# liulisixin/MLI-NeRF

Hardware: AMD Instinct MI355X
Metric: rays/sec + PSNR, syn_hotdog 4096 rays x128 samples, 1/2/4/8 MI355X (higher is better)
Workload: dtype fp16; 1 GPU; syn_hotdog_b stage-b train step; rays_per_gpu=4096, samples_per_ray=128, global_rays=4096, parallelism=dp1, pipeline=geometry prefetch on a side stream, gate heads, 2 batch(es) ahead, output_layer_dw=forward partials (pq), tail=fused, reductions=ordered

## Files before the change

mli_nerf_amd/csrc/params.hip:

```cpp
#include "common.h"

namespace {

__global__ __launch_bounds__(256) void row_scale_kernel(const mli_pack_layer* layers, float* row_scale) {
  const mli_pack_layer& L = layers[blockIdx.y];
  const int row = blockIdx.x * 4 + (threadIdx.x >> 6), lane = threadIdx.x & 63;
  if (row >= L.n_out) return;
  const float* vr = L.v + (size_t)row * L.k_ref;
  float ss = 0.f;
  for (int k = lane; k < L.k_ref; k += 64) ss += vr[k] * vr[k];
#pragma unroll
  for (int o = 32; o > 0; o >>= 1) ss += __shfl_xor(ss, o);
  if (lane == 0) row_scale[blockIdx.y * 256 + row] = L.g[row] / sqrtf(ss);
}

__global__ __launch_bounds__(256) void pack_kernel(const mli_pack_layer* layers, uint8_t* dst,
                                                   const float* row_scale) {
  const mli_pack_layer& L = layers[blockIdx.y];
  const float* rs = row_scale + blockIdx.y * 256;
  const int per_tile = (L.k_steps + 1) * 64;
  const int gid = blockIdx.x * blockDim.x + threadIdx.x;
  if (gid >= L.n_tiles * per_tile) return;
  const int t = gid / per_tile, rem = gid - t * per_tile;
  const int q = rem >> 6, lane = rem & 63;
  uint8_t* chunk = dst + L.dst_offset + (size_t)t * L.chunk_stride;
  const int rows_src = L.n_out, cols_src = L.k_ref;
  if (q == L.k_steps) {
    if (lane >= 32) return;
    const int hh = lane >> 4, i = lane & 15;
    const int n = 32 * t + acc_row(i, hh);
    float b = 0.f;
    if (!L.transpose && L.bias && n < rows_src) b = L.bias[n];
    reinterpret_cast<float*>(chunk + L.k_steps * 1024)[hh * 16 + i] = b;
    return;
  }
  const int rl = lane & 31, hh = lane >> 5;
  const int n = 32 * t + rl;
  half8 out;
  const float sc_row = (!L.transpose && n < rows_src) ? rs[n] : 0.f;
#pragma unroll
  for (int j = 0; j < 8; ++j) {
    const int kk = L.kmode[q] ? k_acc(q, hh, j) : k_nat(q, hh, j);
    const int src = L.kmap[kk];
    float w = 0.f;
    if (src >= 0) {
      if (!L.transpose) {
        if (n < rows_src) w = L.v[(size_t)n * cols_src + src] * sc_row;
      } else {
        const int col = L.nmap ? L.nmap[n] : (n < cols_src ? n : -1);
        if (col >= 0) w = L.v[(size_t)src * cols_src + col] * rs[src];
      }
    }
    out[j] = (f16)w;
  }
  *reinterpret_cast<half8*>(chunk + q * 1024 + lane * 16) = out;
}

__global__ __launch_bounds__(256) void assemble_kernel(const mli_assemble_layer* layers, float inv_scale,
                                                       int zero_dw) {
  const mli_assemble_layer& L = layers[blockIdx.y];
  const int n = blockIdx.x;
  if (n >= L.n_out) return;
  __shared__ float red[2][256];
  const int tid = threadIdx.x;
  float* dwz = const_cast<float*>(L.dw);
  if (L.plain) {
    for (int c = tid; c < L.k_ref; c += 256) {
      const size_t i = (size_t)n * L.k_pack + L.kinv[c];
      L.grad_v[(size_t)n * L.k_ref + c] = L.dw[i] * inv_scale;
      if (zero_dw) dwz[i] = 0.f;
    }
    if (tid == 0) {
      L.grad_b[n] = L.db[n] * inv_scale;
      if (zero_dw) const_cast<float*>(L.db)[n] = 0.f;
    }
    return;
  }
  const float* vr = L.v + (size_t)n * L.k_ref;
  float ss = 0.f, dot = 0.f;
  for (int c = tid; c < L.k_ref; c += 256) {
    const float d = L.dw[(size_t)n * L.k_pack + L.kinv[c]] * inv_scale;
    ss += vr[c] * vr[c];
    dot += d * vr[c];
  }
  red[0][tid] = ss;
  red[1][tid] = dot;
  __syncthreads();
  for (int s = 128; s > 0; s >>= 1) {
    if (tid < s) {
      red[0][tid] += red[0][tid + s];
      red[1][tid] += red[1][tid + s];
    }
    __syncthreads();
  }
  const float nrm = sqrtf(red[0][0]);
  const float dg = red[1][0] / nrm;
  const float gs = L.g[n] / nrm;
  for (int c = tid; c < L.k_ref; c += 256) {
    const size_t i = (size_t)n * L.k_pack + L.kinv[c];
    const float d = L.dw[i] * inv_scale;
    L.grad_v[(size_t)n * L.k_ref + c] = gs * (d - dg * vr[c] / nrm);
    if (zero_dw) dwz[i] = 0.f;
  }
  if (tid == 0) {
    L.grad_g[n] = dg;
    L.grad_b[n] = L.db[n] * inv_scale;
    if (zero_dw) const_cast<float*>(L.db)[n] = 0.f;
  }
}

struct AdamwCoef {
  float decay, omb1, beta2, omb2, step_size, bc2_sqrt, eps;
};

__device__ __forceinline__ void adamw_one(const AdamwCoef& c, float& p, float g, float& m, float& v) {
  p = p * c.decay;
  m = m + (g - m) * c.omb1;
  v = v * c.beta2 + (g * g) * c.omb2;
  const float denom = sqrtf(v) / c.bc2_sqrt + c.eps;
  p = p - c.step_size * (m / denom);
}

__global__ __launch_bounds__(256) void adamw_kernel(mli_adamw_args a, AdamwCoef c) {
  const int64_t i = (int64_t)blockIdx.x * blockDim.x + threadIdx.x;
  if (i >= a.n) return;
  float p = a.p[i], m = a.m[i], v = a.v[i];
  const float g = a.g[i];
  adamw_one(c, p, g, m, v);
  a.p[i] = p;
  a.m[i] = m;
  a.v[i] = v;
  if (a.p16) a.p16[i] = __builtin_bit_cast(uint16_t, (f16)p);
  if (a.zero_grad && g != 0.0f) a.g[i] = 0.0f;
}

__global__ __launch_bounds__(256) void cast_kernel(mli_cast_args a) {
  const int64_t i = (int64_t)blockIdx.x * blockDim.x + threadIdx.x;
  if (i >= a.n) return;
  a.dst[i] = __builtin_bit_cast(uint16_t, (f16)a.src[i]);
}

}

extern "C" int mli_pack(const mli_pack_args* a, mli_stream_t s) {
  const int max_threads = 8 * (19 + 1) * 64;
  if (a->n_layers <= 0) return 0;
  if (a->row_scale == nullptr) return (int)hipErrorInvalidValue;
  hipLaunchKernelGGL(row_scale_kernel, dim3(64, a->n_layers), dim3(256), 0, (hipStream_t)s, a->layers,
                     a->row_scale);
  hipLaunchKernelGGL(pack_kernel, dim3((max_threads + 255) / 256, a->n_layers), dim3(256), 0,
                     (hipStream_t)s, a->layers, a->dst, (const float*)a->row_scale);
  MLI_LAUNCH_CHECK();
}

extern "C" int mli_pack_workspace(const mli_pack_args* a, int64_t* bytes) {
  bytes[0] = (int64_t)(a->n_layers > 0 ? a->n_layers : 0) * 256 * 4;
  return 0;
}

extern "C" int mli_grad_assemble(const mli_assemble_args* a, mli_stream_t s) {
  hipLaunchKernelGGL(assemble_kernel, dim3(256, a->n_layers), dim3(256), 0, (hipStream_t)s,
                     a->layers, a->inv_scale, a->zero_dw);
  MLI_LAUNCH_CHECK();
}

extern "C" int mli_adamw(const mli_adamw_args* a, mli_stream_t s) {
  if (a->n <= 0) return 0;
  const double bc1 = 1.0 - pow(a->beta1, (double)a->step);
  const double bc2 = 1.0 - pow(a->beta2, (double)a->step);
  const AdamwCoef c = {(float)(1.0 - a->lr * a->weight_decay), (float)(1.0 - a->beta1), (float)a->beta2,
                       (float)(1.0 - a->beta2), (float)(a->lr / bc1), (float)sqrt(bc2), (float)a->eps};
  hipLaunchKernelGGL(adamw_kernel, dim3((unsigned)((a->n + 255) / 256)), dim3(256), 0, (hipStream_t)s, *a, c);
  MLI_LAUNCH_CHECK();
}

extern "C" int mli_cast_f16(const mli_cast_args* a, mli_stream_t s) {
  if (a->n <= 0) return 0;
  hipLaunchKernelGGL(cast_kernel, dim3((unsigned)((a->n + 255) / 256)), dim3(256), 0, (hipStream_t)s, *a);
  MLI_LAUNCH_CHECK();
}

extern "C" int mli_abi_version(void) { return MLI_ABI_VERSION; }

#ifndef MLI_SOURCE_HASH
#define MLI_SOURCE_HASH "unknown"
#endif
static const char mli_source_hash_tag[] __attribute__((used)) = "MLI_SOURCE_HASH=" MLI_SOURCE_HASH;
extern "C" const char* mli_source_hash(void) { return mli_source_hash_tag + 16; }

extern "C" const char* mli_error_string(int code) { return hipGetErrorString((hipError_t)code); }
```

mli_nerf_amd/csrc/rays.hip:

```cpp
#include "common.h"
#include "loss.h"
#include "mli_relight.h"

namespace {

MLI_FI float light_pos(const float* Q, int i) {
  return -((Q[4 * 0 + i] * Q[3] + Q[4 * 1 + i] * Q[7]) + Q[4 * 2 + i] * Q[11]);
}

__global__ __launch_bounds__(256) void rays_kernel(mli_rays_args a) {
  const int r = blockIdx.x * blockDim.x + threadIdx.x;
  if (r >= a.R) return;
  const int64_t pix = a.ray_idx ? a.ray_idx[r] : a.first_pixel + r;
  const float py = (float)(pix / a.W) + 0.5f;
  const float px = (float)(pix % a.W) + 0.5f;
  float K[9], T[12], TL[3];
  {
    const float* M = a.intr;
    const float c00 = M[4] * M[8] - M[5] * M[7], c01 = M[5] * M[6] - M[3] * M[8], c02 = M[3] * M[7] - M[4] * M[6];
    const float det = (M[0] * c00 + M[1] * c01) + M[2] * c02;
    const float id = 1.0f / det;
    K[0] = c00 * id; K[1] = (M[2] * M[7] - M[1] * M[8]) * id; K[2] = (M[1] * M[5] - M[2] * M[4]) * id;
    K[3] = c01 * id; K[4] = (M[0] * M[8] - M[2] * M[6]) * id; K[5] = (M[2] * M[3] - M[0] * M[5]) * id;
    K[6] = c02 * id; K[7] = (M[1] * M[6] - M[0] * M[7]) * id; K[8] = (M[0] * M[4] - M[1] * M[3]) * id;
// ... 455 lines not shown
  for (int o = 16; o > 0; o >>= 1) t += __shfl_xor(t, o);
  if (j == 0) fin[i] = t;
  __syncthreads();
  if (threadIdx.x == 0) mli_loss::finalize(L, fin);
}

__global__ __launch_bounds__(256) void composite_bwd_kernel(mli_composite_bwd_args a) {
  const int R = a.R;
  const size_t S = (size_t)R * a.N;
  const size_t s = (size_t)blockIdx.x * 256 + threadIdx.x;
  if (s >= S) return;
  const int r = (int)(s % (size_t)R);
  float dr[3], dor[3], dre[3], orr[3];
  for (int i = 0; i < 3; ++i) {
    dre[i] = a.d_o_re ? a.d_o_re[3 * r + i] : 0.f;
    dr[i] = a.d_rgb ? a.d_rgb[3 * r + i] : 0.f;
    dor[i] = a.d_o_r ? a.d_o_r[3 * r + i] : 0.f;
    orr[i] = a.o_r[3 * r + i];
  }
  const float dos = a.d_o_s ? a.d_o_s[r] : 0.f;
  const f32x4 y0 = *reinterpret_cast<const f32x4*>(a.y + 8 * s);
  const f32x4 y1 = *reinterpret_cast<const f32x4*>(a.y + 8 * s + 4);
  const float y[7] = {y0[0], y0[1], y0[2], y0[3], y1[0], y1[1], y1[2]};
  float D[7];
  ray_dz(dr, dor, dos, dre, orr, a.o_s[r], D);
  if (a.dray && s < (size_t)R) store_dray(a.dray, r, D);
  f32x4 o0, o1;
  composite_bwd_sample(D, a.weights[s] * a.grad_scale, y, o0, o1);
  *reinterpret_cast<f32x4*>(a.dz4 + 8 * s) = o0;
  *reinterpret_cast<f32x4*>(a.dz4 + 8 * s + 4) = o1;
}


__global__ __launch_bounds__(CW * 64) void composite_bwd_geo_kernel(mli_composite_bwd_geo_args a) {
  const int lane = threadIdx.x & 63, w = threadIdx.x >> 6;
  const int R = a.R, N = a.N;
  const int r = blockIdx.x * CW + w;
  if (r >= R) return;
  const float inv_s = expf(a.s_var[0]);
  const float an = a.anneal;
  const float v0 = a.ray_unit[3 * r], v1 = a.ray_unit[3 * r + 1], v2 = a.ray_unit[3 * r + 2];
  const float far = a.far_[r];
  const float dr0 = a.d_rgb[3 * r], dr1 = a.d_rgb[3 * r + 1], dr2 = a.d_rgb[3 * r + 2];
  const float bg = a.white_bg ? (dr0 + dr1) + dr2 : 0.f;
  constexpr int E = 4;
  float al[E], x[E], cp[E], cn[E], ep[E], en[E], st[E], cs[E], dw[E], yv[E][3];
  float lp = 1.f;
#pragma unroll
  for (int e = 0; e < E; ++e) {
    const int k = E * lane + e;
    al[e] = 0.f; x[e] = 0.f; cp[e] = cn[e] = 0.5f; ep[e] = en[e] = 0.f; st[e] = 0.f; cs[e] = 0.f; dw[e] = 0.f;
    yv[e][0] = yv[e][1] = yv[e][2] = 0.f;
    if (k < N) {
      const size_t s = (size_t)k * R + r;
      const float dk = a.dists[s];
      const float dn = (k + 1 < N) ? a.dists[s + R] : far;
      st[e] = dn - dk;
      const float g0 = a.grad[3 * s], g1 = a.grad[3 * s + 1], g2 = a.grad[3 * s + 2];
      cs[e] = (v0 * g0 + v1 * g1) + v2 * g2;
      const float ic = -(fmaxf(-cs[e] * 0.5f + 0.5f, 0.f) * (1.0f - an) + fmaxf(-cs[e], 0.f) * an);
      const float sd = a.sdf[s];
      ep[e] = sd - (ic * st[e]) * 0.5f;
      en[e] = sd + (ic * st[e]) * 0.5f;
      cp[e] = 1.0f / (1.0f + expf(-(ep[e] * inv_s)));
      cn[e] = 1.0f / (1.0f + expf(-(en[e] * inv_s)));
      x[e] = (cp[e] - cn[e]) / (cp[e] + 1e-5f);
      al[e] = fminf(fmaxf(x[e], 0.f), 1.f);
      const f32x4 y0 = *reinterpret_cast<const f32x4*>(a.y + 8 * s);
      yv[e][0] = y0[0]; yv[e][1] = y0[1]; yv[e][2] = y0[2];
      dw[e] = ((dr0 * y0[0] + dr1 * y0[1]) + dr2 * y0[2]) - bg;
    }
    lp *= 1.0f - al[e];
  }
  float T[E];
  T[0] = wave_excl_prod(lp, lane);
#pragma unroll
  for (int e = 1; e < E; ++e) T[e] = T[e - 1] * (1.0f - al[e - 1]);
  float ma = 1.f, mb = 0.f;
#pragma unroll
  for (int e = E - 1; e >= 0; --e) {
    mb = (1.0f - al[e]) * mb + dw[e] * al[e];
    ma = (1.0f - al[e]) * ma;
  }
#pragma unroll
  for (int o = 1; o < 64; o <<= 1) {
    const float na = __shfl_down(ma, o), nb = __shfl_down(mb, o);
    if (lane + o < 64) { mb = ma * nb + mb; ma = ma * na; }
  }
  float B = __shfl_down(mb, 1);
  if (lane == 63) B = 0.f;
  float dinv = 0.f;
#pragma unroll
  for (int e = E - 1; e >= 0; --e) {
    const int k = E * lane + e;
    const float da = T[e] * (dw[e] - B);
    B = (1.0f - al[e]) * B + dw[e] * al[e];
    if (k >= N) continue;
    const size_t s = (size_t)k * R + r;
    const float dx = (x[e] >= 0.f && x[e] <= 1.f) ? da : 0.f;
    const float den_ = cp[e] + 1e-5f;
    const float dcp = dx * (1.0f - x[e]) / den_, dcn = -dx / den_;
    const float dtp = dcp * (cp[e] * (1.0f - cp[e])), dtn = dcn * (cn[e] * (1.0f - cn[e]));
    const float dep = dtp * inv_s, den = dtn * inv_s;
    dinv += dtp * ep[e] + dtn * en[e];
    a.d_sdf[s] = dep + den;
    const float dic = (den - dep) * 0.5f * st[e];
    const float dcos = dic * ((-cs[e] * 0.5f + 0.5f > 0.f ? 0.5f * (1.0f - an) : 0.f) + (-cs[e] > 0.f ? an : 0.f));
    a.d_grad[3 * s] = v0 * dcos;
    a.d_grad[3 * s + 1] = v1 * dcos;
    a.d_grad[3 * s + 2] = v2 * dcos;
    const float wsc = al[e] * T[e] * a.grad_scale;
    f32x4 o0, o1;
    o0[0] = wsc * dr0 * (yv[e][0] * (1.f - yv[e][0]));
    o0[1] = wsc * dr1 * (yv[e][1] * (1.f - yv[e][1]));
    o0[2] = wsc * dr2 * (yv[e][2] * (1.f - yv[e][2]));
    o0[3] = 0.f;
    o1[0] = o1[1] = o1[2] = o1[3] = 0.f;
    *reinterpret_cast<f32x4*>(a.dz4 + 8 * s) = o0;
    *reinterpret_cast<f32x4*>(a.dz4 + 8 * s + 4) = o1;
  }
  dinv = wave_sum(dinv);
  if (lane == 0) a.d_inv_s_part[r] = dinv;
}

__global__ __launch_bounds__(256) void svar_grad_kernel(mli_composite_bwd_geo_args a) {
  __shared__ float red[256];
  float t = 0.f;
  for (int r = threadIdx.x; r < a.R; r += 256) t += a.d_inv_s_part[r];
  red[threadIdx.x] = t;
  __syncthreads();
  for (int o = 128; o > 0; o >>= 1) {
    if ((int)threadIdx.x < o) red[threadIdx.x] += red[threadIdx.x + o];
    __syncthreads();
  }
  if (threadIdx.x == 0) a.d_s_var[0] = expf(a.s_var[0]) * red[0];
}


MLI_FI uint32_t mix32(uint32_t x) {
  x ^= x >> 16; x *= 0x7feb352du; x ^= x >> 15; x *= 0x846ca68bu; x ^= x >> 16;
  return x;
}

MLI_FI uint64_t feistel(uint64_t x, int bits, uint64_t seed) {
  const int lb = bits >> 1, hb = bits - lb;
  const uint64_t lmask = (1ull << lb) - 1ull, hmask = (1ull << hb) - 1ull;
  uint64_t L = x >> lb, Rr = x & lmask;
  for (int k = 0; k < 4; ++k) {
    const uint32_t f = mix32((uint32_t)Rr ^ mix32((uint32_t)(seed >> (8 * k)) + 0x9e3779b9u * (k + 1)) ^
                             (uint32_t)(seed >> 32));
    const uint64_t nL = Rr, nR = (L ^ f) & hmask;
    const uint64_t comb = (nL << hb) | nR;
    L = comb >> lb;
    Rr = comb & lmask;
  }
  return (L << lb) | Rr;
}

__global__ __launch_bounds__(256) void ray_batch_kernel(mli_ray_batch_args a) {
  const int r = blockIdx.x * blockDim.x + threadIdx.x;
  if (r >= a.R) return;
  int bits = 1;
  while ((1ll << bits) < a.n_pixels) ++bits;
  uint64_t x = (uint64_t)r;
  do {
    x = feistel(x, bits, a.seed);
  } while (x >= (uint64_t)a.n_pixels);
  const int64_t p = (int64_t)x, n = a.n_pixels;
  a.ray_idx[r] = p;
  if (a.image)
    for (int c = 0; c < 3; ++c) a.image_sampled[3 * r + c] = a.image[c * n + p];
  if (a.ref)
    for (int c = 0; c < 3; ++c) a.ref_sampled[3 * r + c] = a.ref[c * n + p];
  if (a.sha) a.sha_sampled[r] = a.sha[p];
  if (a.cert) a.cert_sampled[r] = a.cert[p];
}

}

extern "C" int mli_rays(const mli_rays_args* a, mli_stream_t s) {
  if (a->R <= 0) return 0;
  hipLaunchKernelGGL(rays_kernel, dim3((a->R + 255) / 256), dim3(256), 0, (hipStream_t)s, *a);
  MLI_LAUNCH_CHECK();
}

extern "C" int mli_light_points(const mli_light_points_args* a, mli_stream_t s) {
  if (a->L <= 0 || a->R <= 0) return 0;
  if (!a->pose_lights || !a->pts_light) return (int)hipErrorInvalidValue;
  if ((int64_t)a->L * a->R > INT32_MAX) return (int)hipErrorInvalidValue;
  const int64_t n = (int64_t)a->L * a->R * 3;
  hipLaunchKernelGGL(light_points_kernel, dim3((unsigned)((n + 255) / 256)), dim3(256), 0, (hipStream_t)s, *a);
  MLI_LAUNCH_CHECK();
}

extern "C" int mli_sample_coarse(const mli_sample_coarse_args* a, mli_stream_t s) {
  const int n = a->R * a->Nc;
  if (n <= 0) return 0;
  hipLaunchKernelGGL(sample_coarse_kernel, dim3((n + 255) / 256), dim3(256), 0, (hipStream_t)s, *a);
  MLI_LAUNCH_CHECK();
}

extern "C" int mli_sample_fine(const mli_sample_fine_args* a, mli_stream_t s) {
  if (a->R <= 0) return 0;
  if (a->Nf > FBMAX || a->Nb > FBMAX || a->Na < 1 || a->Na + a->Nb > FMAX) return (int)hipErrorInvalidValue;
  if (a->Nf > 0 && a->sdf_out == nullptr) return (int)hipErrorInvalidValue;
  if ((a->inside_list == nullptr) != (a->n_inside == nullptr)) return (int)hipErrorInvalidValue;
  FineArgs fa;
  fa.a = *a;
  for (int j = 0; j < 64; ++j) fa.u[j] = (j < a->Nf && a->u_fine) ? a->u_fine[j] : 2.0f;
  hipLaunchKernelGGL(sample_fine_kernel, dim3((a->R + FW - 1) / FW), dim3(FW * 64), 0, (hipStream_t)s, fa);
  MLI_LAUNCH_CHECK();
}

extern "C" int mli_composite_fwd(const mli_composite_args* a, mli_stream_t s) {
  if (a->R <= 0) return 0;
  if (a->N > 256) return (int)hipErrorInvalidValue;
  if (a->N <= 32 * CE)
    hipLaunchKernelGGL(composite_fwd_kernel<32>, dim3((a->R + 2 * CW - 1) / (2 * CW)), dim3(CW * 64), 0,
                       (hipStream_t)s, *a);
  else
    hipLaunchKernelGGL(composite_fwd_kernel<64>, dim3((a->R + CW - 1) / CW), dim3(CW * 64), 0, (hipStream_t)s, *a);
  MLI_LAUNCH_CHECK();
}

extern "C" int mli_composite_bwd(const mli_composite_bwd_args* a, mli_stream_t s) {
  if (a->R <= 0) return 0;
  const size_t S = (size_t)a->R * a->N;
  hipLaunchKernelGGL(composite_bwd_kernel, dim3((unsigned)((S + 255) / 256)), dim3(256), 0, (hipStream_t)s, *a);
  MLI_LAUNCH_CHECK();
}

extern "C" int mli_composite_bwd_geo(const mli_composite_bwd_geo_args* a, mli_stream_t s) {
  if (a->R <= 0) return 0;
  if (a->N > 256) return (int)hipErrorInvalidValue;
  if (a->d_inv_s_part == nullptr) return (int)hipErrorInvalidValue;
  hipLaunchKernelGGL(composite_bwd_geo_kernel, dim3((a->R + CW - 1) / CW), dim3(CW * 64), 0, (hipStream_t)s, *a);
  hipLaunchKernelGGL(svar_grad_kernel, dim3(1), dim3(256), 0, (hipStream_t)s, *a);
  MLI_LAUNCH_CHECK();
}

extern "C" int mli_composite_bwd_geo_workspace(const mli_composite_bwd_geo_args* a, int64_t* bytes) {
  if (a->R <= 0 || a->N <= 0) return (int)hipErrorInvalidValue;
  const int64_t S = (int64_t)a->R * a->N;
  bytes[0] = S * 8 * 4;
  bytes[1] = S * 4;
  bytes[2] = S * 3 * 4;
  bytes[3] = (int64_t)a->R * 4;
  return 0;
}

extern "C" int mli_ray_batch(const mli_ray_batch_args* a, mli_stream_t s) {
  if (a->R <= 0) return 0;
  if (a->n_pixels < a->R || a->n_pixels > (1ll << 40) || !a->ray_idx) return (int)hipErrorInvalidValue;
  hipLaunchKernelGGL(ray_batch_kernel, dim3((a->R + 255) / 256), dim3(256), 0, (hipStream_t)s, *a);
  MLI_LAUNCH_CHECK();
}

struct CLGeo {
  int rpb, nb;
};
static CLGeo cl_geo(int R, int N) {
  const int rpb = N <= 32 * CE ? 2 * CW : CW;
  return CLGeo{rpb, (R + rpb - 1) / rpb};
}
static bool cl_valid(const mli_composite_loss_args* a) {
  const mli_composite_args& c = a->comp;
  const mli_loss_args& l = a->loss;
  if (c.R <= 0 || c.N <= 0 || c.N > 256 || l.R != c.R || l.N != c.N) return false;
  if (!c.weights || !c.rgb || !c.o_r || !c.o_s || !c.o_re || !a->dz4 || !l.scratch || !l.losses || !l.gt ||
      !l.outside || !c.y)
    return false;
  return !(l.w_intrinsic != 0.f && (l.sha == nullptr || l.cert == nullptr || l.ref == nullptr));
}

extern "C" int mli_composite_loss(const mli_composite_loss_args* a, mli_stream_t s) {
  if (!cl_valid(a)) return (int)hipErrorInvalidValue;
  const CLGeo g = cl_geo(a->comp.R, a->comp.N);
  if (g.rpb == 2 * CW)
    hipLaunchKernelGGL(composite_loss_kernel<32>, dim3(g.nb), dim3(CW * 64), 0, (hipStream_t)s, *a);
  else
    hipLaunchKernelGGL(composite_loss_kernel<64>, dim3(g.nb), dim3(CW * 64), 0, (hipStream_t)s, *a);
  if (!a->defer_finalize)
    hipLaunchKernelGGL(composite_loss_finalize, dim3(1), dim3(256), 0, (hipStream_t)s, a->loss, g.nb);
  MLI_LAUNCH_CHECK();
}

extern "C" int mli_composite_loss_finalize(const mli_composite_loss_args* a, mli_stream_t s) {
  if (!cl_valid(a)) return (int)hipErrorInvalidValue;
  hipLaunchKernelGGL(composite_loss_finalize, dim3(1), dim3(256), 0, (hipStream_t)s, a->loss,
                     cl_geo(a->comp.R, a->comp.N).nb);
  MLI_LAUNCH_CHECK();
}

extern "C" int mli_composite_loss_workspace(const mli_composite_loss_args* a, int64_t* bytes) {
  const int R = a->comp.R;
  if (R <= 0 || a->comp.N <= 0) return (int)hipErrorInvalidValue;
  bytes[0] = (int64_t)mli_loss::ACC_N * cl_geo(R, a->comp.N).nb * 4;
  bytes[1] = (int64_t)R * a->comp.N * 8 * 4;
  return 0;
}

namespace {

constexpr int LR_RAYS = 64, LR_SCAN = 1024;

__global__ __launch_bounds__(4 * LR_RAYS) void live_flags_kernel(mli_live_rays_args a) {
  __shared__ int any[4][LR_RAYS];
  const int rl = threadIdx.x % LR_RAYS, j = threadIdx.x / LR_RAYS;
  const int r = blockIdx.x * LR_RAYS + rl;
  int live = 0;
  if (r < a.R)
    for (int k = j; k < a.N; k += 4)
      live |= (__builtin_bit_cast(uint32_t, a.weights[(size_t)k * a.R + r]) & 0x7fffffffu) != 0;
  any[j][rl] = live;
  __syncthreads();
  live = any[0][rl] | any[1][rl] | any[2][rl] | any[3][rl];
  if (r >= a.R) return;
  if (j == 0) a.flags[r] = live;
  if (!live && a.y != nullptr) {
    const f32x4 z = {0.f, 0.f, 0.f, 0.f};
    for (int k = j; k < a.N; k += 4) {
      f32x4* row = reinterpret_cast<f32x4*>(a.y + ((size_t)k * a.R + r) * 8);
      row[0] = z;
      row[1] = z;
    }
  }
}

template <bool TILES, class Flag, class Emit>
MLI_FI void compact_scan(int n, Flag flag, Emit emit, int& kept, int& bits) {
  __shared__ int sums[1 + TILES][LR_SCAN];
  const int t = threadIdx.x;
  const int per = (n + LR_SCAN - 1) / LR_SCAN;
  const int r0 = min(t * per, n), r1 = min(r0 + per, n);
  int cnt = 0, wcnt = 0;
  for (int r = r0; r < r1; ++r) {
    const uint32_t f = flag(r);
    cnt += f != 0;
    if (TILES) wcnt += __popc(f);
  }
  sums[0][t] = cnt;
  if (TILES) sums[TILES][t] = wcnt;
  __syncthreads();
  for (int o = 1; o < LR_SCAN; o <<= 1) {
    const int v = t >= o ? sums[0][t - o] : 0, wv = TILES && t >= o ? sums[TILES][t - o] : 0;
    __syncthreads();
    sums[0][t] += v;
    if (TILES) sums[TILES][t] += wv;
    __syncthreads();
  }
  kept = sums[0][LR_SCAN - 1];
  bits = TILES ? sums[TILES][LR_SCAN - 1] : 0;
  int before = sums[0][t] - cnt;
  int wbefore = TILES ? sums[TILES][t] - wcnt : 0;
  for (int r = r0; r < r1; ++r) {
    const uint32_t f = flag(r);
    emit(r, f, f != 0 ? before : kept + (r - before), before, wbefore);
    before += f != 0;
    if (TILES) wbefore += __popc(f);
  }
}

__global__ __launch_bounds__(LR_SCAN) void live_scan_kernel(mli_live_rays_args a) {
  const int T = a.N / 32, G = 256 / a.N;
  int L, none;
  compact_scan<false>(
      a.R, [&](int r) MLI_LAMBDA_FI { return (uint32_t)a.flags[r]; },
      [&](int r, uint32_t live, int pos, int before, int) MLI_LAMBDA_FI {
        for (int i = 0; i < T; ++i) {
          a.tile_list[pos * T + i] = r * T + i;
          a.tile_rank[r * T + i] = before * T + (live ? i : 0);
        }
      },
      L, none);
  if (threadIdx.x == 0) {
    a.tile_rank[a.R * T] = L * T;
    a.n_live_tiles[0] = (L + G - 1) / G * G * T;
  }
}

}

extern "C" int mli_live_rays(const mli_live_rays_args* a, mli_stream_t s) {
  if (a->R <= 0 || a->N <= 0 || a->N % 32 != 0 || 256 % a->N != 0 || a->R % (256 / a->N) != 0)
    return (int)hipErrorInvalidValue;
  if (!a->weights || !a->flags || !a->tile_list || !a->tile_rank || !a->n_live_tiles) return (int)hipErrorInvalidValue;
  hipLaunchKernelGGL(live_flags_kernel, dim3((a->R + LR_RAYS - 1) / LR_RAYS), dim3(4 * LR_RAYS), 0, (hipStream_t)s, *a);
  hipLaunchKernelGGL(live_scan_kernel, dim3(1), dim3(LR_SCAN), 0, (hipStream_t)s, *a);
  MLI_LAUNCH_CHECK();
}

namespace {

__global__ __launch_bounds__(LR_SCAN) void inside_list_kernel(mli_inside_list_args a, int fill_blocks) {
  const int t = threadIdx.x;
  if ((int)blockIdx.x < fill_blocks) {
    const size_t i = (size_t)blockIdx.x * LR_SCAN + t;
    if (i >= (size_t)a.R * a.N) return;
    const int r = (int)(i % a.R);
    if (!a.outside[r]) return;
    if (a.dists != nullptr) {
      const float near = a.near_[r], far = a.far_[r];
      const float d = near + (((float)(i / a.R) + 0.5f) / (float)a.N) * (far - near);
      a.dists[i] = fminf(fmaxf(d, near), far);
    }
    if (a.sdf == nullptr) return;
    a.sdf[i] = a.outside_val;
    a.grad[3 * i] = 0.0f;
    a.grad[3 * i + 1] = 0.0f;
    a.grad[3 * i + 2] = 0.0f;
    if (a.hess != nullptr) {
      a.hess[3 * i] = 0.0f;
      a.hess[3 * i + 1] = 0.0f;
      a.hess[3 * i + 2] = 0.0f;
    }
    return;
  }
  int n_in, none;
  compact_scan<false>(
      a.R, [&](int r) MLI_LAMBDA_FI { return (uint32_t)(a.outside[r] == 0); },
      [&](int r, uint32_t, int pos, int, int) MLI_LAMBDA_FI { a.inside_list[pos] = r; }, n_in, none);
  if (t == 0) a.n_inside[0] = min(n_in + a.n_pad, a.R);
}

}

extern "C" int mli_inside_list(const mli_inside_list_args* a, mli_stream_t s) {
  if (a->R <= 0 || a->N <= 0 || a->n_pad < 0 || !a->outside || !a->inside_list || !a->n_inside)
    return (int)hipErrorInvalidValue;
  if ((a->sdf == nullptr) != (a->grad == nullptr) || (a->hess != nullptr && a->sdf == nullptr))
    return (int)hipErrorInvalidValue;
  if ((a->dists == nullptr) != (a->near_ == nullptr) || (a->dists == nullptr) != (a->far_ == nullptr))
    return (int)hipErrorInvalidValue;
  const int64_t S = (int64_t)a->R * a->N;
  const int fill_blocks = (a->sdf || a->dists) ? (int)((S + LR_SCAN - 1) / LR_SCAN) : 0;
  hipLaunchKernelGGL(inside_list_kernel, dim3(fill_blocks + 1), dim3(LR_SCAN), 0, (hipStream_t)s, *a, fill_blocks);
  MLI_LAUNCH_CHECK();
}

namespace {

constexpr int LT_WAVES = LR_SCAN / 64;

MLI_FI void live_tiles_scan(const mli_live_tiles_args& a) {
  const int R = a.comp.R, N = a.comp.N;
  const int T = N / 32, G = 256 / N;
  int L, W;
  compact_scan<true>(
      R,
      [&](int r) MLI_LAMBDA_FI {
        return (uint32_t)__hip_atomic_load(a.flags + r, __ATOMIC_RELAXED, __HIP_MEMORY_SCOPE_AGENT);
      },
      [&](int r, uint32_t f, int pos, int before, int wbefore) MLI_LAMBDA_FI {
        for (int i = 0; i < T; ++i) {
          const int below = wbefore + __popc(f & ((1u << i) - 1u));
          a.tile_list[pos * T + i] = r * T + i;
          a.tile_rank[r * T + i] = before * T + (f != 0 ? i : 0);
          a.wtile_rank[pos * T + i] = f != 0 ? below : W;
          if ((f >> i) & 1u) {
            a.wtile_list[below] = pos * T + i;
          } else if (a.n_wtiles_pad != nullptr) {
            const int z = pos * T + i - (f != 0 ? below : W);
            if (z < ((8 - (W & 7)) & 7)) a.wtile_list[W + z] = pos * T + i;
          }
        }
      },
      L, W);
  if (threadIdx.x == 0) {
    a.tile_rank[R * T] = L * T;
    a.wtile_rank[R * T] = W;
    a.n_live_tiles[0] = (L + G - 1) / G * G * T;
    if (a.n_wtiles_pad != nullptr) a.n_wtiles_pad[0] = (W + 7) & ~7;
  }
}

template <int L>
__global__ __launch_bounds__(LR_SCAN) void live_tiles_kernel(mli_live_tiles_args a) {
  __shared__ int last;
  const int lane = threadIdx.x & 63, w = threadIdx.x >> 6;
  const int sub = lane % L;
  const int r = (blockIdx.x * LT_WAVES + w) * (64 / L) + lane / L;
  const int R = a.comp.R, N = a.comp.N;
  if (r < R) {
    float wv[CE], yk[CE][7], acc[12];
    composite_ray<L>(a.comp, r, sub, wv, yk, acc);
    int nz = 0;
#pragma unroll
    for (int e = 0; e < CE; ++e)
      if (CE * sub + e < N) nz |= (__builtin_bit_cast(uint32_t, wv[e]) & 0x7fffffffu) != 0;
    const uint64_t seg = __ballot(nz) >> (lane / L * L);
    uint32_t f = 0;
#pragma unroll
    for (int j = 0; j < L * CE / 32; ++j)
      if (j * 32 < N && ((seg >> (j * (32 / CE))) & ((1u << (32 / CE)) - 1u)) != 0) f |= 1u << j;
    if (sub == 0) a.flags[r] = (int)f;
    if (a.y != nullptr && (f == 0 || a.n_wtiles_pad != nullptr)) {
      const f32x4 z = {0.f, 0.f, 0.f, 0.f};
#pragma unroll
      for (int e = 0; e < CE; ++e) {
        const int k = CE * sub + e;
        if (k < N && ((f >> (k >> 5)) & 1u) == 0) {
          f32x4* row = reinterpret_cast<f32x4*>(a.y + ((size_t)k * R + r) * 8);
          row[0] = z;
          row[1] = z;
        }
      }
    }
  }
  if (a.scan_launch) return;
  __threadfence();
  __syncthreads();
  if (threadIdx.x == 0) last = atomicAdd(a.ticket, 1) == (int)gridDim.x - 1;
  __syncthreads();
  if (!last) return;
  __threadfence();
  live_tiles_scan(a);
  if (threadIdx.x == 0) atomicExch(a.ticket, 0);
}

__global__ __launch_bounds__(LR_SCAN) void live_tiles_scan_kernel(mli_live_tiles_args a) { live_tiles_scan(a); }

}

extern "C" int mli_live_tiles(const mli_live_tiles_args* a, mli_stream_t s) {
  const int R = a->comp.R, N = a->comp.N;
  if (R <= 0 || N <= 0 || N % 32 != 0 || 256 % N != 0 || R % (256 / N) != 0) return (int)hipErrorInvalidValue;
  if (a->comp.y != nullptr || !a->comp.weights || !a->flags || !a->tile_list || !a->tile_rank || !a->n_live_tiles ||
      !a->wtile_list || !a->wtile_rank || (!a->scan_launch && !a->ticket))
    return (int)hipErrorInvalidValue;
  if (N <= 32 * CE) {
    const int rpb = 2 * LT_WAVES;
    hipLaunchKernelGGL(live_tiles_kernel<32>, dim3((R + rpb - 1) / rpb), dim3(LR_SCAN), 0, (hipStream_t)s, *a);
  } else {
    hipLaunchKernelGGL(live_tiles_kernel<64>, dim3((R + LT_WAVES - 1) / LT_WAVES), dim3(LR_SCAN), 0, (hipStream_t)s, *a);
  }
  if (a->scan_launch) hipLaunchKernelGGL(live_tiles_scan_kernel, dim3(1), dim3(LR_SCAN), 0, (hipStream_t)s, *a);
  MLI_LAUNCH_CHECK();
}
```

Before: 2.576 million rays/s.

## Fuse row-scale into pack kernel and rewrite live-ray scans with wave shuffles

The weight-norm row scale computation is folded into the pack kernel, which computes scales into shared memory for just the rows its block needs, removing one launch and a global round trip. The compaction scan drops from a 1024-thread shared-memory Hillis-Steele scan to a 256-thread scan using wave shuffles plus a per-wave total. Flags are cached in registers and loaded as vectors, and tile lists are written as int4 stores when N is 128. The live-tiles kernel block size shrinks with LR_SCAN, and the per-block redundant row-scale work plus the more complex pack indexing could add cost.

```diff
diff --git a/mli_nerf_amd/csrc/params.hip b/mli_nerf_amd/csrc/params.hip
--- a/mli_nerf_amd/csrc/params.hip
+++ b/mli_nerf_amd/csrc/params.hip
@@ -2,56 +2,102 @@
 
 namespace {
 
-__global__ __launch_bounds__(256) void row_scale_kernel(const mli_pack_layer* layers, float* row_scale) {
+constexpr int PK_RB = 16;
+MLI_FI void row_scales(const mli_pack_layer& L, const int (&row)[PK_RB], float* sc, int lane) {
+  const float* vr[PK_RB];
+  float ss[PK_RB], g[PK_RB];
+#pragma unroll
+  for (int b = 0; b < PK_RB; ++b) {
+    const int r = row[b] < 0 ? 0 : row[b];
+    vr[b] = L.v + (size_t)r * L.k_ref;
+    g[b] = L.g[r];
+    ss[b] = 0.f;
+  }
+  for (int k = lane; k < L.k_ref; k += 64) {
+#pragma unroll
+    for (int b = 0; b < PK_RB; ++b) ss[b] += vr[b][k] * vr[b][k];
+  }
+#pragma unroll
+  for (int o = 32; o > 0; o >>= 1) {
+#pragma unroll
+    for (int b = 0; b < PK_RB; ++b) ss[b] += __shfl_xor(ss[b], o);
+  }
+#pragma unroll
+  for (int b = 0; b < PK_RB; ++b)
+    if (lane == 0 && row[b] >= 0) sc[row[b]] = g[b] / sqrtf(ss[b]);
+}
+
+__global__ __launch_bounds__(256) void pack_kernel(const mli_pack_layer* layers, uint8_t* dst) {
+  __shared__ float rs[256];
   const mli_pack_layer& L = layers[blockIdx.y];
-  const int row = blockIdx.x * 4 + (threadIdx.x >> 6), lane = threadIdx.x & 63;
-  if (row >= L.n_out) return;
-  const float* vr = L.v + (size_t)row * L.k_ref;
-  float ss = 0.f;
-  for (int k = lane; k < L.k_ref; k += 64) ss += vr[k] * vr[k];
-#pragma unroll
-  for (int o = 32; o > 0; o >>= 1) ss += __shfl_xor(ss, o);
-  if (lane == 0) row_scale[blockIdx.y * 256 + row] = L.g[row] / sqrtf(ss);
-}
-
-__global__ __launch_bounds__(256) void pack_kernel(const mli_pack_layer* layers, uint8_t* dst,
-                                                   const float* row_scale) {
-  const mli_pack_layer& L = layers[blockIdx.y];
-  const float* rs = row_scale + blockIdx.y * 256;
   const int per_tile = (L.k_steps + 1) * 64;
-  const int gid = blockIdx.x * blockDim.x + threadIdx.x;
-  if (gid >= L.n_tiles * per_tile) return;
+  const int total = L.n_tiles * per_tile;
+  const int gid0 = blockIdx.x * blockDim.x, gid = gid0 + threadIdx.x;
+  if (gid0 >= total) return;
+  const int rows_src = L.n_out, cols_src = L.k_ref;
   const int t = gid / per_tile, rem = gid - t * per_tile;
   const int q = rem >> 6, lane = rem & 63;
-  uint8_t* chunk = dst + L.dst_offset + (size_t)t * L.chunk_stride;
-  const int rows_src = L.n_out, cols_src = L.k_ref;
-  if (q == L.k_steps) {
-    if (lane >= 32) return;
-    const int hh = lane >> 4, i = lane & 15;
-    const int n = 32 * t + acc_row(i, hh);
-    float b = 0.f;
-    if (!L.transpose && L.bias && n < rows_src) b = L.bias[n];
-    reinterpret_cast<float*>(chunk + L.k_steps * 1024)[hh * 16 + i] = b;
-    return;
-  }
   const int rl = lane & 31, hh = lane >> 5;
   const int n = 32 * t + rl;
+  uint8_t* chunk = dst + L.dst_offset + (size_t)t * L.chunk_stride;
+  const bool frag = gid < total && q < L.k_steps;
+  const int qs = frag ? q : 0, ns = frag ? n : 0;
+  int src[8], col, krow;
+  {
+    const int mode = L.kmode[qs];
+    int sa[8], sn[8];
+#pragma unroll
+    for (int j = 0; j < 8; ++j) {
+      sa[j] = L.kmap[k_acc(qs, hh, j)];
+      sn[j] = L.kmap[k_nat(qs, hh, j)];
+    }
+    krow = L.kmap[16 * qs + (lane & 15)];
+    const int nm = L.transpose && L.nmap ? L.nmap[ns] : (ns < cols_src ? ns : -1);
+#pragma unroll
+    for (int j = 0; j < 8; ++j) src[j] = mode ? sa[j] : sn[j];
+    col = !L.transpose ? (ns < rows_src ? ns : -1) : nm;
+  }
+  if (gid < total && q == L.k_steps && lane < 32) {
+    const int bh = lane >> 4, i = lane & 15;
+    const int bn = 32 * t + acc_row(i, bh);
+    float b = 0.f;
+    if (!L.transpose && L.bias && bn < rows_src) b = L.bias[bn];
+    reinterpret_cast<float*>(chunk + L.k_steps * 1024)[bh * 16 + i] = b;
+  }
+  float val[8];
+  int sidx[8];
+#pragma unroll
+  for (int j = 0; j < 8; ++j) {
+    const bool held = frag && src[j] >= 0 && col >= 0;
+    const size_t at = L.transpose ? (size_t)src[j] * cols_src + col : (size_t)col * cols_src + src[j];
+    val[j] = L.v[held ? at : 0];
+    sidx[j] = held ? (L.transpose ? src[j] : col) : -1;
+  }
+  {
+    const int w = threadIdx.x >> 6;
+    int row[PK_RB];
+    if (!L.transpose) {
+      const int lo = 32 * (gid0 / per_tile);
+      const int hi = min(32 * ((min(gid0 + (int)blockDim.x, total) - 1) / per_tile + 1), L.n_out);
+      for (int base = lo + w * PK_RB; base < hi; base += 4 * PK_RB) {
+#pragma unroll
+        for (int b = 0; b < PK_RB; ++b) row[b] = base + b < hi ? base + b : -1;
+        row_scales(L, row, rs, lane);
+      }
+    } else if (__builtin_amdgcn_readfirstlane((int)frag)) {
+#pragma unroll
+      for (int b = 0; b < PK_RB; ++b) row[b] = __builtin_amdgcn_readlane(krow, b);
+      row_scales(L, row, rs, lane);
+    }
+  }
+  __syncthreads();
+  if (!frag) return;
   half8 out;
-  const float sc_row = (!L.transpose && n < rows_src) ? rs[n] : 0.f;
 #pragma unroll
   for (int j = 0; j < 8; ++j) {
-    const int kk = L.kmode[q] ? k_acc(q, hh, j) : k_nat(q, hh, j);
-    const int src = L.kmap[kk];
-    float w = 0.f;
-    if (src >= 0) {
-      if (!L.transpose) {
-        if (n < rows_src) w = L.v[(size_t)n * cols_src + src] * sc_row;
-      } else {
-        const int col = L.nmap ? L.nmap[n] : (n < cols_src ? n : -1);
-        if (col >= 0) w = L.v[(size_t)src * cols_src + col] * rs[src];
-      }
-    }
-    out[j] = (f16)w;
+    float w = val[j] * rs[sidx[j] >= 0 ? sidx[j] : 0];
+    tie(w);
+    out[j] = (f16)(sidx[j] >= 0 ? w : 0.f);
   }
   *reinterpret_cast<half8*>(chunk + q * 1024 + lane * 16) = out;
 }
@@ -146,10 +192,8 @@
   const int max_threads = 8 * (19 + 1) * 64;
   if (a->n_layers <= 0) return 0;
   if (a->row_scale == nullptr) return (int)hipErrorInvalidValue;
-  hipLaunchKernelGGL(row_scale_kernel, dim3(64, a->n_layers), dim3(256), 0, (hipStream_t)s, a->layers,
-                     a->row_scale);
   hipLaunchKernelGGL(pack_kernel, dim3((max_threads + 255) / 256, a->n_layers), dim3(256), 0,
-                     (hipStream_t)s, a->layers, a->dst, (const float*)a->row_scale);
+                     (hipStream_t)s, a->layers, a->dst);
   MLI_LAUNCH_CHECK();
 }
 
diff --git a/mli_nerf_amd/csrc/rays.hip b/mli_nerf_amd/csrc/rays.hip
--- a/mli_nerf_amd/csrc/rays.hip
+++ b/mli_nerf_amd/csrc/rays.hip
@@ -781,7 +781,7 @@
 
 namespace {
 
-constexpr int LR_RAYS = 64, LR_SCAN = 1024;
+constexpr int LR_RAYS = 64, LR_SCAN = 256;
 
 __global__ __launch_bounds__(4 * LR_RAYS) void live_flags_kernel(mli_live_rays_args a) {
   __shared__ int any[4][LR_RAYS];
@@ -806,46 +806,123 @@
   }
 }
 
-template <bool TILES, class Flag, class Emit>
-MLI_FI void compact_scan(int n, Flag flag, Emit emit, int& kept, int& bits) {
-  __shared__ int sums[1 + TILES][LR_SCAN];
-  const int t = threadIdx.x;
+constexpr int LR_REG = 16;
+constexpr int LR_FLAG_BITS = 8, LR_MAX_N = 256;
+static_assert(LR_MAX_N / 32 <= LR_FLAG_BITS, "a ray's tile bits fit one byte of the register path");
+typedef int i32x4 __attribute__((ext_vector_type(4)));
+
+struct ScanFlagsI32 {
+  const int32_t* p;
+  int agent;
+  MLI_FI uint32_t at(int r) const {
+    return agent ? (uint32_t)__hip_atomic_load(p + r, __ATOMIC_RELAXED, __HIP_MEMORY_SCOPE_AGENT) : (uint32_t)p[r];
+  }
+  MLI_FI bool aligned(int r0) const { return !agent && ((uintptr_t)(p + r0) & 15) == 0; }
+  MLI_FI void load16(int r0, uint32_t (&f)[LR_REG]) const {
+    const i32x4* q = reinterpret_cast<const i32x4*>(p + r0);
+#pragma unroll
+    for (int v = 0; v < LR_REG / 4; ++v) {
+      const i32x4 x = q[v];
+#pragma unroll
+      for (int j = 0; j < 4; ++j) f[4 * v + j] = (uint32_t)x[j];
+    }
+  }
+};
+struct ScanFlagsInside {
+  const uint8_t* outside;
+  MLI_FI uint32_t at(int r) const { return (uint32_t)(outside[r] == 0); }
+  MLI_FI bool aligned(int r0) const { return ((uintptr_t)(outside + r0) & 15) == 0; }
+  MLI_FI void load16(int r0, uint32_t (&f)[LR_REG]) const {
+    const u32x4 x = *reinterpret_cast<const u32x4*>(outside + r0);
+#pragma unroll
+    for (int i = 0; i < LR_REG; ++i) f[i] = (uint32_t)(((x[i >> 2] >> (8 * (i & 3))) & 0xffu) == 0);
+  }
+};
+
+template <bool TILES, class Src, class Emit>
+MLI_FI void compact_scan(int n, Src src, Emit emit, int& kept, int& bits) {
+  __shared__ int tot[2][LR_SCAN / 64];
+  const int t = threadIdx.x, lane = t & 63, w = t >> 6;
   const int per = (n + LR_SCAN - 1) / LR_SCAN;
   const int r0 = min(t * per, n), r1 = min(r0 + per, n);
+  const bool reg = per <= LR_REG;
+  uint64_t flo = 0, fhi = 0;
   int cnt = 0, wcnt = 0;
+  if (reg) {
+    uint32_t f[LR_REG];
+    if (r1 - r0 == LR_REG && src.aligned(r0)) {
+      src.load16(r0, f);
+    } else {
+#pragma unroll
+      for (int i = 0; i < LR_REG; ++i) f[i] = r0 + i < r1 ? src.at(r0 + i) : 0u;
+    }
+#pragma unroll
+    for (int i = 0; i < LR_REG; ++i) {
+      cnt += f[i] != 0;
+      if (TILES) wcnt += __popc(f[i]);
+      if (i < 8) flo |= (uint64_t)f[i] << (8 * i);
+      else fhi |= (uint64_t)f[i] << (8 * (i - 8));
+    }
+  } else {
+    for (int r = r0; r < r1; ++r) {
+      const uint32_t f = src.at(r);
+      cnt += f != 0;
+      if (TILES) wcnt += __popc(f);
+    }
+  }
+  int inc = cnt, winc = wcnt;
+#pragma unroll
+  for (int o = 1; o < 64; o <<= 1) {
+    const int v = __shfl_up(inc, o), wv = TILES ? __shfl_up(winc, o) : 0;
+    if (lane >= o) {
+      inc += v;
+      winc += wv;
+    }
+  }
+  if (lane == 63) {
+    tot[0][w] = inc;
+    tot[1][w] = winc;
+  }
+  __syncthreads();
+  int before = inc - cnt;
+  int wbefore = TILES ? winc - wcnt : 0;
+  kept = 0;
+  bits = 0;
+#pragma unroll
+  for (int i = 0; i < LR_SCAN / 64; ++i) {
+    const int c = tot[0][i], wc = TILES ? tot[1][i] : 0;
+    if (i < w) {
+      before += c;
+      wbefore += wc;
+    }
+    kept += c;
+    bits += wc;
+  }
   for (int r = r0; r < r1; ++r) {
-    const uint32_t f = flag(r);
-    cnt += f != 0;
-    if (TILES) wcnt += __popc(f);
-  }
-  sums[0][t] = cnt;
-  if (TILES) sums[TILES][t] = wcnt;
-  __syncthreads();
-  for (int o = 1; o < LR_SCAN; o <<= 1) {
-    const int v = t >= o ? sums[0][t - o] : 0, wv = TILES && t >= o ? sums[TILES][t - o] : 0;
-    __syncthreads();
-    sums[0][t] += v;
-    if (TILES) sums[TILES][t] += wv;
-    __syncthreads();
-  }
-  kept = sums[0][LR_SCAN - 1];
-  bits = TILES ? sums[TILES][LR_SCAN - 1] : 0;
-  int before = sums[0][t] - cnt;
-  int wbefore = TILES ? sums[TILES][t] - wcnt : 0;
-  for (int r = r0; r < r1; ++r) {
-    const uint32_t f = flag(r);
+    const int i = r - r0;
+    const uint32_t f = reg ? (uint32_t)((i < 8 ? flo >> (8 * i) : fhi >> (8 * (i - 8))) & 0xffu) : src.at(r);
     emit(r, f, f != 0 ? before : kept + (r - before), before, wbefore);
     before += f != 0;
     if (TILES) wbefore += __popc(f);
   }
 }
 
-__global__ __launch_bounds__(LR_SCAN) void live_scan_kernel(mli_live_rays_args a) {
+inline int lists_vec4(int N, const void* p0, const void* p1, const void* p2) {
+  return N == 128 && (((uintptr_t)p0 | (uintptr_t)p1 | (uintptr_t)p2) & 15) == 0;
+}
+
+__global__ __launch_bounds__(LR_SCAN) void live_scan_kernel(mli_live_rays_args a, int vec4) {
   const int T = a.N / 32, G = 256 / a.N;
   int L, none;
   compact_scan<false>(
-      a.R, [&](int r) MLI_LAMBDA_FI { return (uint32_t)a.flags[r]; },
+      a.R, ScanFlagsI32{a.flags, 0},
       [&](int r, uint32_t live, int pos, int before, int) MLI_LAMBDA_FI {
+        if (vec4) {
+          const i32x4 iota = {0, 1, 2, 3}, zero = {0, 0, 0, 0};
+          *reinterpret_cast<i32x4*>(a.tile_list + pos * 4) = r * 4 + iota;
+          *reinterpret_cast<i32x4*>(a.tile_rank + r * 4) = before * 4 + (live ? iota : zero);
+          return;
+        }
         for (int i = 0; i < T; ++i) {
           a.tile_list[pos * T + i] = r * T + i;
           a.tile_rank[r * T + i] = before * T + (live ? i : 0);
@@ -865,7 +942,8 @@
     return (int)hipErrorInvalidValue;
   if (!a->weights || !a->flags || !a->tile_list || !a->tile_rank || !a->n_live_tiles) return (int)hipErrorInvalidValue;
   hipLaunchKernelGGL(live_flags_kernel, dim3((a->R + LR_RAYS - 1) / LR_RAYS), dim3(4 * LR_RAYS), 0, (hipStream_t)s, *a);
-  hipLaunchKernelGGL(live_scan_kernel, dim3(1), dim3(LR_SCAN), 0, (hipStream_t)s, *a);
+  hipLaunchKernelGGL(live_scan_kernel, dim3(1), dim3(LR_SCAN), 0, (hipStream_t)s, *a,
+                     lists_vec4(a->N, a->tile_list, a->tile_rank, nullptr));
   MLI_LAUNCH_CHECK();
 }
 
@@ -897,7 +975,7 @@
   }
   int n_in, none;
   compact_scan<false>(
-      a.R, [&](int r) MLI_LAMBDA_FI { return (uint32_t)(a.outside[r] == 0); },
+      a.R, ScanFlagsInside{a.outside},
       [&](int r, uint32_t, int pos, int, int) MLI_LAMBDA_FI { a.inside_list[pos] = r; }, n_in, none);
   if (t == 0) a.n_inside[0] = min(n_in + a.n_pad, a.R);
 }
@@ -919,29 +997,43 @@
 
 namespace {
 
-constexpr int LT_WAVES = LR_SCAN / 64;
-
-MLI_FI void live_tiles_scan(const mli_live_tiles_args& a) {
+constexpr int LT_WAVES = 4;
+static_assert(LT_WAVES * 64 == LR_SCAN, "the last-ticket workgroup scans with its own threads");
+
+MLI_FI void live_tiles_scan(const mli_live_tiles_args& a, int vec4) {
   const int R = a.comp.R, N = a.comp.N;
   const int T = N / 32, G = 256 / N;
   int L, W;
   compact_scan<true>(
-      R,
-      [&](int r) MLI_LAMBDA_FI {
-        return (uint32_t)__hip_atomic_load(a.flags + r, __ATOMIC_RELAXED, __HIP_MEMORY_SCOPE_AGENT);
-      },
+      R, ScanFlagsI32{a.flags, !a.scan_launch},
       [&](int r, uint32_t f, int pos, int before, int wbefore) MLI_LAMBDA_FI {
-        for (int i = 0; i < T; ++i) {
-          const int below = wbefore + __popc(f & ((1u << i) - 1u));
-          a.tile_list[pos * T + i] = r * T + i;
-          a.tile_rank[r * T + i] = before * T + (f != 0 ? i : 0);
-          a.wtile_rank[pos * T + i] = f != 0 ? below : W;
+        const auto wtile = [&](int i, int below) MLI_LAMBDA_FI {
           if ((f >> i) & 1u) {
             a.wtile_list[below] = pos * T + i;
           } else if (a.n_wtiles_pad != nullptr) {
             const int z = pos * T + i - (f != 0 ? below : W);
             if (z < ((8 - (W & 7)) & 7)) a.wtile_list[W + z] = pos * T + i;
           }
+        };
+        if (vec4) {
+          i32x4 below;
+#pragma unroll
+          for (int i = 0; i < 4; ++i) {
+            below[i] = wbefore + __popc(f & ((1u << i) - 1u));
+            wtile(i, below[i]);
+          }
+          const i32x4 iota = {0, 1, 2, 3}, zero = {0, 0, 0, 0}, allw = {W, W, W, W};
+          *reinterpret_cast<i32x4*>(a.tile_list + pos * 4) = r * 4 + iota;
+          *reinterpret_cast<i32x4*>(a.tile_rank + r * 4) = before * 4 + (f != 0 ? iota : zero);
+          *reinterpret_cast<i32x4*>(a.wtile_rank + pos * 4) = f != 0 ? below : allw;
+          return;
+        }
+        for (int i = 0; i < T; ++i) {
+          const int below = wbefore + __popc(f & ((1u << i) - 1u));
+          a.tile_list[pos * T + i] = r * T + i;
+          a.tile_rank[r * T + i] = before * T + (f != 0 ? i : 0);
+          a.wtile_rank[pos * T + i] = f != 0 ? below : W;
+          wtile(i, below);
         }
       },
       L, W);
@@ -954,7 +1046,7 @@
 }
 
 template <int L>
-__global__ __launch_bounds__(LR_SCAN) void live_tiles_kernel(mli_live_tiles_args a) {
+__global__ __launch_bounds__(LR_SCAN) void live_tiles_kernel(mli_live_tiles_args a, int vec4) {
   __shared__ int last;
   const int lane = threadIdx.x & 63, w = threadIdx.x >> 6;
   const int sub = lane % L;
@@ -993,26 +1085,31 @@
   __syncthreads();
   if (!last) return;
   __threadfence();
-  live_tiles_scan(a);
+  live_tiles_scan(a, vec4);
   if (threadIdx.x == 0) atomicExch(a.ticket, 0);
 }
 
-__global__ __launch_bounds__(LR_SCAN) void live_tiles_scan_kernel(mli_live_tiles_args a) { live_tiles_scan(a); }
+__global__ __launch_bounds__(LR_SCAN) void live_tiles_scan_kernel(mli_live_tiles_args a, int vec4) {
+  live_tiles_scan(a, vec4);
+}
 
 }
 
 extern "C" int mli_live_tiles(const mli_live_tiles_args* a, mli_stream_t s) {
   const int R = a->comp.R, N = a->comp.N;
-  if (R <= 0 || N <= 0 || N % 32 != 0 || 256 % N != 0 || R % (256 / N) != 0) return (int)hipErrorInvalidValue;
+  if (R <= 0 || N <= 0 || N % 32 != 0 || LR_MAX_N % N != 0 || R % (LR_MAX_N / N) != 0) return (int)hipErrorInvalidValue;
   if (a->comp.y != nullptr || !a->comp.weights || !a->flags || !a->tile_list || !a->tile_rank || !a->n_live_tiles ||
       !a->wtile_list || !a->wtile_rank || (!a->scan_launch && !a->ticket))
     return (int)hipErrorInvalidValue;
+  const int vec4 = lists_vec4(N, a->tile_list, a->tile_rank, a->wtile_rank);
   if (N <= 32 * CE) {
     const int rpb = 2 * LT_WAVES;
-    hipLaunchKernelGGL(live_tiles_kernel<32>, dim3((R + rpb - 1) / rpb), dim3(LR_SCAN), 0, (hipStream_t)s, *a);
+    hipLaunchKernelGGL(live_tiles_kernel<32>, dim3((R + rpb - 1) / rpb), dim3(LR_SCAN), 0, (hipStream_t)s, *a, vec4);
   } else {
-    hipLaunchKernelGGL(live_tiles_kernel<64>, dim3((R + LT_WAVES - 1) / LT_WAVES), dim3(LR_SCAN), 0, (hipStream_t)s, *a);
-  }
-  if (a->scan_launch) hipLaunchKernelGGL(live_tiles_scan_kernel, dim3(1), dim3(LR_SCAN), 0, (hipStream_t)s, *a);
-  MLI_LAUNCH_CHECK();
-}
+    hipLaunchKernelGGL(live_tiles_kernel<64>, dim3((R + LT_WAVES - 1) / LT_WAVES), dim3(LR_SCAN), 0, (hipStream_t)s, *a,
+                       vec4);
+  }
+  if (a->scan_launch)
+    hipLaunchKernelGGL(live_tiles_scan_kernel, dim3(1), dim3(LR_SCAN), 0, (hipStream_t)s, *a, vec4);
+  MLI_LAUNCH_CHECK();
+}
```

New measurement: 2.562 million rays/s. No clear change (-0.6%).
